# Blaok/soda

Hardware: AMD Instinct MI355X
Metric: stencil cells*iters/s, jacobi2d 8192x8192 iterate=100 (higher is better)
Workload: dtype f32; 1 GPU; jacobi2d float 8192x8192 iterate=100; kernel_family=march2d, decomposition=none, overlap=False, transport=none

## Files before the change

### soda_amd/codegen/hip/lower.py

```python
import dataclasses
import os
from typing import Dict, Optional, Sequence, Union

from soda_amd import core, util

from soda_amd.codegen.hip.module import (KernelDesc, Module, PassDesc,
                                         _check_native, runtime_text)
from soda_amd.codegen.hip.direct import DIRECT_BLOCK, add_direct_pass
from soda_amd.codegen.hip.ldswin import (add_ldswin_pass,
                                         ldswin_candidate, ldswin_pays,
                                         ldswin_supported)
from soda_amd.codegen.hip.march import (LANE_SHIFTS, MAX_FUSE_3D,
                                        MAX_FUSE_PRESERVE, MAX_SHIFT_TEMPS,
                                        MAX_UNROLL, REG_BUDGET, MarchConfig,
                                        add_march_pass, default_vec,
                                        march_supported)


MAX_TENSORS = 16
DEFAULT_FUSE = (13, 12, 8, 4)
SLIDING_SUMS = os.environ.get('SODA_HIP_SLIDE', '1') != '0'


STRATEGIES = ('auto', 'direct', 'march', 'ldswin')


@dataclasses.dataclass(kw_only=True, eq=False)
class LowerOptions:

  strategy: str = 'auto'
  fuse: Sequence[int] = (4,)
  vec: Optional[int] = None
  chunk_rows: Optional[int] = None
  prefetch: Optional[int] = None
  waves_x: int = 1
  waves_y: int = 1
  nt_store: Optional[bool] = None
  nt_load: Optional[bool] = None
  xcd_swizzle: bool = True
  edge_loads: bool = True
  tile_rows: Optional[int] = None
  lane_shift: Optional[str] = None
  min_waves: int = 0
  occupancy: int = 0
  pipe: Optional[int] = None
  pipe_rows: int = 2
  reg_budget: Optional[int] = None
  stamps: bool = False
  peel: Union[None, int, Dict[int, int]] = None
  align_lanes: Optional[int] = None
  xshare: Optional[bool] = None
  row_cells: Optional[int] = None
  windows: Optional[bool] = None
  inline: Optional[bool] = None

  def __post_init__(self):
    self.fuse = tuple(self.fuse)
    if self.inline is None:
      self.inline = os.environ.get('SODA_HIP_INLINE', '1') != '0'
    if self.windows is None:
      self.windows = os.environ.get('SODA_HIP_WINDOWS', '1') != '0'
    if self.xshare is None and os.environ.get('SODA_HIP_XSHARE'):
      self.xshare = os.environ['SODA_HIP_XSHARE'] == '1'
    if self.align_lanes is None and os.environ.get('SODA_HIP_ALIGN_LANES'):
      self.align_lanes = int(os.environ['SODA_HIP_ALIGN_LANES'])

  def resolved(self, dim: int, iterated: bool = True) -> 'LowerOptions':
    out = dataclasses.replace(self)
    if out.prefetch is None and dim == 3:
      out.prefetch = 1
    if out.nt_load is None:
      out.nt_load = dim != 3 and iterated
    if out.nt_store is None:
      out.nt_store = not iterated
    if out.tile_rows is None:
      out.tile_rows = 4
    return out


NARROW_STRIP_OPS = (48, 128)


def prefers_narrow_strips(stencil: core.Stencil) -> bool:
  if os.environ.get('SODA_HIP_NARROW', '1') == '0':
    return False
  if stencil.dim != 2 or stencil.iterate != 1:
    return False
  if any(str(t) != 'float' for t in stencil.symbol_table.values()):
    return False
  from soda_amd import ir as _ir
  work = sum(_ir.op_count(s.stmt.expr) +
             sum(_ir.op_count(l.expr) for l in s.stmt.let)
             for s in stencil.ordered_stages)
  return NARROW_STRIP_OPS[0] <= work < NARROW_STRIP_OPS[1]


# ... 66 lines not shown
    skip = ()
    if marching:
      skip = ((0, None),) + (((stencil.dim - 1, '+'),) if SLIDING_SUMS else ())
    derived = windows.decompose(stencil, skip=skip)
    if len(derived.symbol_table) + len(derived.param_stmts) <= MAX_TENSORS \
        and same_boxes(derived):
      stencil = derived
  from soda_amd.codegen.hip import exact
  stencil = exact.specialize(stencil)
  mod = Module(stencil)
  use_march = opts.strategy in ('auto', 'march') and \
      march_supported(stencil) is None
  if opts.strategy == 'march' and not use_march:
    raise util.SemanticError('march: %s' % march_supported(stencil))
  if use_march:
    vec0 = opts.vec or default_vec(stencil)
    iterable = (len(stencil.input_names) == len(stencil.output_names) and
                stencil.input_types == stencil.output_types)
    cap = stencil.iterate
    if stencil.dim == 3 and opts.strategy != 'march':
      cap = min(cap, MAX_FUSE_3D)
    if stencil.preserve_border and opts.strategy != 'march':
      cap = min(cap, MAX_FUSE_PRESERVE)
    depths = sorted({min(t, cap) for t in opts.fuse if iterable} - {0, 1},
                    reverse=True)

    def peel_for(t: int) -> int:
      if opts.peel is None:
        return -1
      if isinstance(opts.peel, dict):
        return int(opts.peel.get(t, -1))
      return int(opts.peel)

    def pipe_for(t: int) -> int:
      want = default_pipe(t) if opts.pipe is None else opts.pipe
      ok = (want > 1 and t > 1 and t % want == 0 and
            opts.waves_x * opts.waves_y == 1)
      return want if ok else 1

    out_bytes = min(t.size_in_bytes for t in stencil.output_types)

    def shift_for(t: int, xshare: int = 0) -> str:
      if opts.lane_shift is not None:
        return opts.lane_shift
      if xshare or pipe_for(t) > 1 or opts.waves_x * opts.waves_y != 1:
        return 'dpp'
      return default_lane_shift(t, stencil.dim)

    def config(t: int, vec: int, pf: Optional[int],
               rows: Optional[int] = None, xshare: int = 0) -> MarchConfig:
      shift = shift_for(t, xshare)
      if pf is None:
        pf = default_prefetch(t, shift)
      if opts.align_lanes is not None:
        align = opts.align_lanes
      else:
        align = max(1, 64 // (vec * out_bytes)) if opts.nt_store else 1
      cfg = MarchConfig(
          fused_iters=t, vec=vec, chunk_rows=opts.chunk_rows or 64,
          prefetch=pf, waves_x=opts.waves_x, waves_y=opts.waves_y,
          nt_store=opts.nt_store, nt_load=opts.nt_load,
          xcd_swizzle=opts.xcd_swizzle, edge_loads=opts.edge_loads,
          tile_rows=rows or opts.tile_rows, lane_shift=shift,
          min_waves=opts.min_waves, occupancy=opts.occupancy,
          pipe=pipe_for(t), pipe_rows=opts.pipe_rows, stamps=opts.stamps,
          peel=peel_for(t), align_lanes=align, xshare=xshare,
          xwindow=bool(opts.windows),
          slide=bool(opts.windows) and SLIDING_SUMS)
      cfg.chunk_fixed = opts.chunk_rows is not None
      return cfg

    budget = opts.reg_budget or REG_BUDGET
    first = default_prefetch(1) if stencil.dim == 2 and work < 128 else \
        (2 if stencil.dim == 2 else 1)
    pfs = [opts.prefetch] if opts.prefetch else [first, 2, 1]
    pfs = sorted(set(pfs), reverse=True)
    rows_list = [opts.tile_rows]
    vecs = []
    v = vec0
    while v >= 1:
      vecs.append(v)
      v //= 2
    chosen = None
    last_error = None
    for v in vecs:
      for rows in rows_list:
        for pf in pfs:
          trial = Module(stencil)
          try:
            est = add_march_pass(trial, config(1, v, pf, rows)).traffic_model[
                'est_window_regs']
          except util.SemanticError as e:
            last_error = e
            continue
          if chosen is None or est < chosen[0]:
            chosen = (est, v, pf, rows)
          if est <= budget:
            break
        if chosen and chosen[0] <= budget:
          break
      if chosen and chosen[0] <= budget:
# ... 38 lines not shown
```

### soda_amd/codegen/hip/march.py

```python
from typing import Dict, List, Optional, Tuple

from soda_amd import core, ir, util

from soda_amd.codegen.hip.module import KernelDesc, Module, PassDesc

MAX_UNROLL = 24
MAX_FUSE_PRESERVE = 8
MAX_FUSE_3D = 2
MAX_SHIFT_TEMPS = 64
REG_BUDGET = 160


class _Node:

  def __init__(self, key, ctype: str, stage: Optional[core.Stage], it: int):
    self.key = key
    self.ctype = ctype
    self.stage = stage
    self.it = it
    self.parents: Dict[str, '_Node'] = {}
    self.delay = 0
    self.first_use = None
    self.window = 1
    self.slots = 1
# ... 6 lines not shown
    self.keep: Optional[str] = None
    self.xs = False

  def tap_bounds(self, pname: str):
    dim = len(self.stage.st_idx)
    if pname in self.stage.taps:
      lo, hi = self.stage.tap_bounds(pname)
    else:
      lo, hi = (0,) * dim, (0,) * dim
    if pname == self.keep:
      lo = tuple(min(0, v) for v in lo)
      hi = tuple(max(0, v) for v in hi)
    return lo, hi

  @property
  def is_input(self) -> bool:
    return self.stage is None and self.mirror_of is None

  @property
  def fill_delay(self) -> int:
    if self.mirror_of is not None:
      return self.delay - MIRROR_PREFETCH
    return 0 if self.stage is None else self.delay

  @property
  def var(self) -> str:
    if self.mirror_of is not None:
      return 'm%d_%s' % (self.owner, self.mirror_of.var)
    if self.stage is None:
      return 'g_%s' % self.key[1]
    return 't%d_%s' % (self.it, self.stage.name)


LDS_PER_CU = 160 * 1024
MIRROR_PREFETCH = 1


LANE_SHIFTS = {'dpp': '', 'mixh': '_mixh'}


class MarchConfig:

  def __init__(self, *, fused_iters: int = 1, vec: int = 4, chunk_rows: int = 64,
               prefetch: int = 2, waves_x: int = 1, waves_y: int = 1,
               nt_store: bool = False, nt_load: bool = True,
               xcd_swizzle: bool = True, edge_loads: bool = True,
               tile_rows: int = 6, lane_shift: str = 'dpp',
               min_waves: int = 0, occupancy: int = 0,
               pipe: int = 1, pipe_rows: int = 4, stamps: bool = False,
               peel: int = -1, align_lanes: int = 1, xshare: int = 0,
               xwindow: bool = True, slide: bool = True):
    self.xwindow = xwindow
    self.slide = slide
    self.xshare = int(xshare)
    self.align_lanes = max(1, int(align_lanes))
    self.peel = int(peel)
    self.stamps = stamps
    self.pipe_rows = pipe_rows if pipe > 1 else 1
    self.pipe = pipe
    self.occupancy = occupancy
    self.min_waves = min_waves
    self.lane_shift = lane_shift
    self.fused_iters = fused_iters
    self.vec = vec
    self.chunk_rows = chunk_rows
    self.prefetch = prefetch
    self.waves_x = waves_x
    self.waves_y = waves_y
    self.nt_store = nt_store
    self.nt_load = nt_load
    self.xcd_swizzle = xcd_swizzle
    self.edge_loads = edge_loads
    self.tile_rows = tile_rows
    self.chunk_fixed = False

  def key(self) -> str:
    return ''.join((
        'T%d_V%d_P%d_W%dx%d_R%d' % (self.fused_iters, self.vec, self.prefetch,
                                    self.waves_x, self.waves_y, self.tile_rows),
        '_nts' if self.nt_store else '', '_ntl' if self.nt_load else '',
        '_xcd' if self.xcd_swizzle else '', '_edge' if self.edge_loads else '',
        LANE_SHIFTS[self.lane_shift],
        '_mw%d' % self.min_waves if self.min_waves else '',
        '_occ%d' % self.occupancy if self.occupancy else '',
        '_buf',
        '_pipe%dx%d' % (self.pipe, self.pipe_rows) if self.pipe > 1 else '',
        '_st' if self.stamps else '',
        '_k%d' % self.peel if self.peel >= 0 else '',
        '_al%d' % self.align_lanes if self.align_lanes > 1 else '',
        '_xs%d' % self.xshare if self.xshare else ''))


def default_vec(stencil: core.Stencil) -> int:
  widest = max(t.size_in_bytes for t in stencil.symbol_table.values())
  return max(1, 16 // widest)


def march_supported(stencil: core.Stencil) -> Optional[str]:
  if stencil.dim not in (2, 3):
    return 'the marching kernels need a 2- or 3-dimensional program'
  return None


def _build_chain(st: core.Stencil, T: int, pf: int, edge: Tuple[int, int],
                 pipe: int = 1, pipe_rows: int = 1, xshare: bool = False):
  dim = st.dim
  ax = dim - 1
  table = st.symbol_table
  per_wave = T // pipe
  nodes: List[_Node] = []
  inputs = {}
  for name in st.input_names:
    n = _Node(('in', name), table[name].c_type, None, -1)
    n.delay = pf
    n.margin = [-edge[0], -edge[1]]
# ... 436 lines not shown
      self.xs_stride = self.xs * 2 * self.xs_rows
      for n in self.xs_nodes:
        self.w('  __shared__ %s soda_xs_%s[%d];' %
               (n.ctype, n.var, 2 * self.xs_stride + 1))
      self.w('  if (threadIdx.x == 0) {')
      for n in self.xs_nodes:
        self.w('    soda_xs_%s[%d] = (%s)0;' % (n.var, 2 * self.xs_stride, n.ctype))
      self.w('  }')
      self.w('  soda_pipe_barrier();')
      self.w('  const int xs_wr = (wave * 2 + (lane == 0 ? 0 : 1)) * %d;' %
             self.xs_rows)
      self.w('  const int xs_nb = lane < 32 ? wave - 1 : wave + 1;')
      self.w('  const int xs_rd = (xs_nb >= 0 && xs_nb < %d && (lane & 31) < %d) ? '
             '(xs_nb * 2 + (lane < 32 ? 1 : 0)) * %d + (lane & 31) : %d;' %
             (self.xs, self.xs_rows, self.xs_rows, 2 * self.xs_stride))
    if self.n_edge:
      for i in range(self.n_edge):
        self.w('  const int ex%d = lane == 0 ? x0 - %d : x0 + %d;' %
          (i, 1 + i, self.V + i))
        self.w('  const bool edge_ok%d = edge_lane && ex%d >= 0 && ex%d < n0;' %
          (i, i, i))
        for es in sorted({self.esz[nme] for nme in self.inputs}):
          self.w('  const unsigned exb%d_%d = edge_ok%d ? (unsigned)ex%d * %du : '
            'SODA_OOB_X;' % (i, es, i, i, es))

    if self.st.preserve_border:
      for o in self.st.output_names:
        wlo, whi = self.st.interior_bounds(o)
        for e in range(self.V):
          self.w('  const bool keepx_%s_%d = !(a.origin[0] + x0 + %d >= %d && '
                 'a.origin[0] + x0 + %d < a.gextent[0] - %d);'
                 % (o, e, e, max(0, -wlo[0]), e, max(0, whi[0])))
    self.use_mix = self.cfg.lane_shift == 'mixh'
    self.slide: Dict[int, Tuple[str, Tuple[int, ...], int]] = {}
    if self.cfg.xwindow and self.cfg.slide and self.W == 1:
      from soda_amd.optimization import windows
      table = dict(self.st.symbol_table)
      for n in self.nodes:
        if n.stage is None or n.mirror_of is not None or n.keep is not None:
          continue
        m = windows._match(n.stage.stmt, table)
        if m is None or m[0] != '+' or m[2] != self.ax:
          continue
        off = tuple(a - b for a, b in zip(m[5], n.stage.st_idx))
        self.slide[id(n)] = (m[1], off, m[4])
    declared = set()
    for stage in self.st.ordered_stages:
      for line in self.mod.param_decls(stage):
        if line not in declared:
          declared.add(line)
          self.w(line)
    for n in self.nodes:
      if n.to_lds:
        self.w('  __shared__ %s soda_ring_%s[%d][%d][%d];' % (
            n.ctype, n.var, 2 * self.R, self.rows_in, 64 * self.V))
    self.nt_l = 'true' if self.cfg.nt_load else 'false'
    self.nt_s = 'true' if self.cfg.nt_store else 'false'

  def emit_decls(self, wv: int) -> None:
      for n in self.nodes:
        if n.owner != wv:
          continue
        if id(n) in self.slide:
          for j in self.rows_of(n):
            self.w('  int xa_%s_r%d[%d];' % (n.var, j, self.V))
            self.w('  soda_zero_frag<int, %d>(xa_%s_r%d);' % (self.V, n.var, j))
# ... 14 lines not shown
      if pin:
        for es in sorted({self.esz[nme] for nme in self.inputs}):
          self.w('      unsigned xb%dp = xb%d; asm volatile("" : "+v"(xb%dp));'
                 % (es, es, es))
      pinned = 'p' if pin else ''
      for es in sorted({self.esz[nme] for nme in self.inputs}):
        if self.dim == 2:
          self.w('      const unsigned ro%d = plane_ok ? (unsigned)(t - wlo) * '
            'pitch_b%d : SODA_OOB_ROW;' % (es, es))
        else:
          self.w('      const unsigned po%d = plane_ok ? (unsigned)(t - wlo) * '
            'pitch_b%d : SODA_OOB_X;' % (es, es))
          for j in sorted({j for n in self.inputs.values() for j in self.rows_of(n)}):
            self.w('      const unsigned ro%d_%d = po%d + yo%d_%d;' %
                   (es, j, es, es, j))
      for nme, n in self.inputs.items():
        s = self.slot_of(n, k, 0)
        for j in self.rows_of(n):
          es = self.esz[nme]
          ro = 'ro%d' % es if self.dim == 2 else 'ro%d_%d' % (es, j)
          reg = '%s_s%d_r%d' % (n.var, s, j)
          self.w('      soda_buf_load_frag<%s, %d, %s>(%s, r_%s, %s + xb%d%s);' %
            (n.ctype, self.V, self.nt_l, reg, nme, ro, es, pinned))
          for i in range(self.n_edge):
            self.w('      { %s e1[1]; soda_buf_load_frag<%s, 1, false>(e1, r_%s, %s + '
              'exb%d_%d); %s_e[%d] = e1[0]; }' %
              (n.ctype, n.ctype, nme, ro, i, es, reg, i))

  def _emit_wave(self, wv: int) -> None:
    if self.W > 1:
      self.w('  if (wave == %d) {  // iterations %d..%d of the chain' %
             (wv, wv * (self.T // self.W), (wv + 1) * (self.T // self.W) - 1))
    self.emit_decls(wv)
    self.w('  int tau = m_begin + (%d);' % (self.m_lo + self.lead))
    if wv == 0:
      for i in range(self.lead):
        self.w('    {  // prologue: loads of plane tau - %d' % (self.lead - i))
        self.emit_loads((i - self.lead) % self.U, 'tau - %d' % (self.lead - i))
        self.w('    }')
    self.w('  const int tau_end = m_end + %d;' % self.max_delay)
    if self.peeled:
      self.w('  {  // warm-up: %d row steps, stages enter as their rows start '
             'to matter' % self.peeled)
      for i in range(self.peeled):
        self._emit_tick(wv, i % self.U, step=i)
      self.w('  }')
      self.w('  tau += %d;' % self.peeled)
    for n in self.nodes:
      if id(n) in self.slide and n.owner == wv and not (
          self.peeled and self.stage_needed(n, self.peeled - 1)):
        self.w('  {  // sliding sum of %s: the rows its window holds now' % n.var)
        self.w('    const int t = tau;')
        self._shifted = {}
        self._wide = {}
        self._stage_mark = len(self.L)
        self._emit_stage(n, 0, slide_init='only')
        self.w('  }')
    self.w('  for (; tau < tau_end; tau += %d) {' % self.U)
    for k in range(self.U):
      self._emit_tick(wv, k)
    self.w('  }')
    if self.W > 1:
      self.w('  }')

  def _emit_tick(self, wv: int, k: int, step: Optional[int] = None) -> None:
    at = k if step is None else step
    self.w('    {  // tick %d of %d' % (k, self.U))

    if self.W > 1 and k % self.R == 0:
      self.w('      soda_pipe_barrier();')
    if wv == 0:
      self.emit_loads(k, 'tau + %d' % at, pin=step is not None)
    else:
      self.w('      const int t = tau + %d;' % at)
    for n in self.nodes:
      if n.mirror_of is not None and n.owner == wv:
        for j in self.rows_of(n):
          self.w('      soda_load_frag<%s, %d, false>(%s_s%d_r%d, &soda_ring_%s'
                 '[(t + %d) & %d][%d][lane * %d]);' %
                 (n.ctype, self.V, n.var, self.slot_of(n, k, 0), j,
                  n.mirror_of.var, self.R, 2 * self.R - 1, j, self.V))
    self._shifted: Dict[Tuple[str, int, int, int, int], str] = {}
    self._wide: Dict[str, str] = {}
    self._stage_mark = len(self.L)
    fresh_xs: List[Tuple[_Node, int]] = []
    if self.xs and wv == 0:
      for n in self.inputs.values():
        if n.xs:
          fresh_xs.append((n, self.slot_of(n, k, self.PF)))
      for n in self.nodes:
        if not n.xs:
          continue
        slot = self.slot_of(n, k - 1, self.PF if n.is_input else 0)
        self.w('      hv_%s_s%d = soda_xs_%s[xs_rd < %d ? xs_rd + ((t - 1) & 1) * %d '
               ': xs_rd];' % (n.var, slot, n.var, 2 * self.xs_stride,
                              self.xs_stride))
    for n in self.nodes:
      if n.stage is not None and n.owner == wv:
        if step is not None and not self.stage_needed(n, step):
          continue
        first = step is not None and (step == 0 or
                                      not self.stage_needed(n, step - 1))
        self._emit_stage(n, k, slide_init='first' if first else None)
        if n.xs:
          fresh_xs.append((n, self.slot_of(n, k, 0)))
    self.shift_temps = max(self.shift_temps, len(self._shifted))
    if fresh_xs:
      self.w('      if (edge_lane) {')
      for n, slot in fresh_xs:
        for jj, j in enumerate(self.rows_of(n)):
          reg = '%s_s%d_r%d' % (n.var, slot, j)
          self.w('        soda_xs_%s[xs_wr + (t & 1) * %d + %d] = lane == 0 ? %s[0] '
                 ': %s[%d];' % (n.var, self.xs_stride, jj, reg, reg, self.V - 1))
      self.w('      }')
      self.w('      soda_pipe_barrier();')
    self.w('    }')

  def _emit_stage(self, n: _Node, k: int,
                  slide_init: Optional[str] = None) -> None:
    stage = n.stage
    pre: List[str] = []
    early: List[str] = []

    def operand(pname: str, off: Tuple[int, ...], j: int, e: int, _n=n,
                _k=k, _pre=pre, _early=early) -> str:
      p = _n.parents[pname]
      age = _n.delay - off[self.ax] - p.fill_delay
      slot = self.slot_of(p, _k, age)
      row = j + (off[1] if self.dim == 3 else 0)
      if row < p.rmargin[0] or row >= self.rows_in - p.rmargin[1]:
        raise util.InternalError('march: row %d of %s is not held' %
                                 (row, p.var))
      reg = '%s_s%d_r%d' % (p.var, slot, row)
      c = e + off[0]
      lane_off, sub = c // self.V, c % self.V
      src = '%s[%d]' % (reg, sub)
      byte = p.ctype in ('uint8_t', 'int8_t')

      def wide(text: str, tag: str) -> str:
        if not byte:
          return text
        if tag not in self._wide:
          self._wide[tag] = 'w%d_%s' % (len(self._wide), tag)
          _pre.append('      const int %s = soda_wide(%s);' %
                      (self._wide[tag], text))
        return self._wide[tag]

      if lane_off == 0:
        return wide(src, '%s_e%d' % (reg, sub))
      key = (p.var, slot, row, sub, lane_off)
      if key not in self._shifted:
        tmp = 'sh_%s_e%d_%s%d' % (reg, sub, 'm' if lane_off < 0 else 'p',
                                  abs(lane_off))
        if (p.is_input and self.n_edge) or p.xs:
          if abs(lane_off) != 1:
            raise util.InternalError('march: edge loads reach one lane')
          ei = (-c - 1) if lane_off < 0 else (c - self.V)
          if p.xs:
            rr = row - p.rmargin[0] + (0 if lane_off < 0 else 32)
            old = ('soda_bcast(hv_%s_s%d, %d)' % (p.var, slot, rr)
                   if ei == 0 else '(%s)0' % p.ctype)
          else:
            old = '%s_e[%d]' % (reg, ei) if 0 <= ei < self.n_edge else \
                '(%s)0' % p.ctype
          expr = ('soda_lane_dn_or(%s, %s)' if lane_off < 0 else
                  'soda_lane_up_or(%s, %s)') % (src, old)
        elif self.use_mix and lane_off > 0:
          expr = src
          for _ in range(lane_off):
            expr = 'soda_lane_up32(%s)' % expr
        else:
          expr = src
          for _ in range(abs(lane_off)):
            expr = ('soda_lane_dn(%s)' if lane_off < 0 else
                    'soda_lane_up(%s)') % expr
        line = '      const %s %s = %s;' % (p.ctype, tmp, expr)
        early = self.use_mix and lane_off > 0 and (
            p.is_input or age > 0) and not (p.is_input and self.n_edge) \
            and not p.xs
        (_early if early else _pre).append(line)
        self._shifted[key] = tmp
      return wide(self._shifted[key], self._shifted[key])
# ... 152 lines not shown
                '%s(%s, (%s)%s)' % (fn, prev, pt, cells[i])
            body.append('        const %s %s = %s;' % (pt, name, expr))
            pre[i] = prev = name
          for e in range(e0, e0 + b):
            parts = ['xm_%s' % btag]
            if e < lo:
              parts.append(suf[e])
            if e + taps - 1 > hi:
              parts.append(pre[e + taps - 1])
            expr = parts[0]
            for q in parts[1:]:
              expr = '%s(%s, %s)' % (fn, expr, q)
            body.append('        %s = (%s)(%s);' % (dst[e], n.ctype, expr))
      body.append('      }')

  def _emit_store(self, n: _Node, oname: str, dst_slot: int) -> None:
    es = self.esz[oname]
    self.w('      {')
    self.w('        const int m = t - %d;' % n.delay)
    self.w('        const bool m_ok = m >= m_begin && m < m_end;')
    for j in self.store_rows(n):
      reg = '%s_s%d_r%d' % (n.var, dst_slot, j)
      if self.dim == 3:
        self.w('        soda_buf_store_frag<%s, %d, %s>(w_%s, (m_ok ? (unsigned)'
          '(m - m_begin) * pitch_b%d : SODA_OOB_X) + yo%d_%d + sxb%d, %s);' %
          (n.ctype, self.V, self.nt_s, oname, es, es, j, es, reg))
      else:
        self.w('        soda_buf_store_frag<%s, %d, %s>(w_%s, (m_ok ? '
          '(unsigned)(m - m_begin) * pitch_b%d : SODA_OOB_ROW) + sxb%d, '
          '%s);' % (n.ctype, self.V, self.nt_s, oname, es, es, reg))
    self.w('      }')

  def _finish(self) -> PassDesc:
    if self.shift_temps > MAX_SHIFT_TEMPS:
      raise util.SemanticError(
          'march: %d lane-shifted operands per row step (> %d); the taps reach '
          'too far along dim 0 for %d cells per lane' %
          (self.shift_temps, MAX_SHIFT_TEMPS, self.V))
    self.est_regs += self.shift_temps
    stages = [n for n in self.nodes if n.stage is not None]
    per_wave = []
    for wv in range(self.W):
      ops = 0.0
      for n in stages:
        if n.owner != wv:
          continue
        cost = sum(ir.op_count(l.expr) for l in n.stage.stmt.let) + \
            ir.op_count(n.stage.stmt.expr) + 0.5
        wide = 2.0 if n.ctype in ('double', 'int64_t', 'uint64_t') else 1.0
        ops += cost * wide * self.V * len(self.rows_of(n))
      per_wave.append(ops + 8.0)
    step_ops = max(per_wave)
    saved = sum(1 for i in range(self.peeled) for n in stages
                if not self.stage_needed(n, i)) / float(max(1, len(stages)))
    if self.dim == 2:
      tile = (self.strip_cells * (self.xs or self.wx),
              self.cfg.chunk_rows * self.cfg.waves_y)
    else:
      tile = (self.strip_cells * (self.xs or 1), self.tile_rows,
              self.cfg.chunk_rows)
    lds_pad = 0
    if self.cfg.occupancy:
      blocks_per_cu = max(1, 4 * self.cfg.occupancy // self.waves)
      lds_pad = min(65536, (LDS_PER_CU // (blocks_per_cu + 1)) // 1024 * 1024
                    + 1024)
    idx = self.mod.add_kernel(
        KernelDesc(self.name, (self.block, 1, 1), tile, lds_bytes=lds_pad,
                   note='%s %s' % (self.kind, self.cfg.key()),
                   tune=dict(axis=self.ax, waves_along=self.cfg.waves_y if self.dim == 2 else 1,
                             waves_per_block=self.waves, warm=self.warm,
                             fixed=self.cfg.chunk_fixed, occupancy=self.cfg.occupancy,
                             pipe=self.W, vec=self.V, step_ops=step_ops,
# ... 32 lines not shown
```

### soda_amd/csrc/soda_hip.cpp

```cpp
#include "soda_internal.h"

#include <hip/hiprtc.h>

#include <cmath>
#include <cstdlib>
#include <cstring>
#include <new>

namespace soda_detail {

thread_local std::string g_error;

int fail(int status, const std::string& what) {
  g_error = what;
  return status;
}

const std::string& last_error_text() { return g_error; }

int hip_fail(hipError_t e, const char* what) {
  char buf[512];
  snprintf(buf, sizeof buf, "%s: %s (%d)", what, hipGetErrorString(e), (int)e);
  g_error = buf;
  if (e == hipErrorOutOfMemory) return SODA_HIP_ERR_NOMEM;
// ... 266 lines not shown
      if (b.ptr) (void)hipFree(b.ptr);
  for (int i = 0; i < 2; ++i) {
    if (p->ev_pre[i]) (void)hipEventDestroy(p->ev_pre[i]);
    if (p->ev_bnd[i]) (void)hipEventDestroy(p->ev_bnd[i]);
  }
  if (p->side) (void)hipStreamDestroy(p->side);
  for (auto& st : p->hstream)
    if (st) (void)hipStreamDestroy(st);
  p->ring_in.release();
  p->ring_out.release();
  for (auto& b : p->band_out)
    if (b.ptr) (void)hipFree(b.ptr);
  for (auto& e : p->hevents) (void)hipEventDestroy(e);
  if (p->module) (void)hipModuleUnload(p->module);
  delete p;
  return SODA_HIP_OK;
}

namespace {

const int kSimds = 1024;
const double kHbmBytesPerNs = 6369.0;
const double kLaunchNs = 2547.0;
const double kWaveNs = 391.0;
const double kNormP = 2.708;
const int64_t kBufWindowMax = 1ll << 30;

int waves_per_simd(int vgprs) {
  int alloc = vgprs < 8 ? 8 : (vgprs + 7) / 8 * 8;
  int w = 512 / alloc;
  return w < 1 ? 1 : w > 8 ? 8 : w;
}

double issue_share(int64_t k) { return k == 1 ? 2.0 : k == 2 ? 1.2 : 1.0; }
double time_share(int64_t k) {
  return k == 1 ? 1.312 : k == 2 ? 1.475 : k == 3 ? 1.365 : 1.046;
}

int32_t tuned_chunk(const soda_hip_kernel_desc_t& d, const int32_t* tile,
                    const int32_t* extent, int dim, int64_t others) {
  const int axis = d.march_dim - 1;
  const int32_t n = extent[axis];
  const int wpb = (d.block[0] * d.block[1] * d.block[2] + 63) / 64;
  const int along = d.waves_along > 0 ? d.waves_along : 1;
  const bool load_only_warm = d.warm > 12 && d.warm_saved >= 0.75 * d.warm;
  const double warm = load_only_warm ? d.warm : d.warm - d.warm_saved;
  (void)tile; (void)dim;
  const int cap = waves_per_simd(d.vgprs);
  if (d.pipe > 1) {
    int32_t target = (int32_t)(3.5 * d.warm) > 64 ? (int32_t)(3.5 * d.warm) : 64;
    int64_t chunks = (n + target - 1) / target;
    if (chunks < 1) chunks = 1;
    const int64_t slots = (int64_t)kSimds * cap / d.pipe;
    int64_t blocks = others * chunks;
    if (blocks > slots * 0.975 && blocks < slots * 1.6) {
      chunks = (int64_t)(slots * 0.975) / others;
      if (chunks < 1) chunks = 1;
    }
    return (int32_t)((n + chunks - 1) / chunks);
  }
  const int k_min = d.warm <= 12 ? 4 : 2;
  double best_cost = 0;
  int32_t best = 0;
  for (int32_t chunk = n < 8 ? n : 8; chunk <= n;) {
    int64_t chunks = (n + chunk - 1) / chunk;
    int64_t blocks = others * ((chunks + along - 1) / along);
    int64_t waves = blocks * wpb;
    double cost;
    const int64_t slots = (int64_t)cap * kSimds;
    if (waves <= slots) {
      int64_t k = (waves + kSimds - 1) / kSimds;
      if (cap > 1) {
        if (k >= cap && waves > 0.975 * k * kSimds) ++k;
        if (k < k_min) k = k_min;
      }
      cost = k * issue_share(k) * (chunk + warm);
    } else {
      const int64_t full = waves / slots, rem = waves - full * slots;
      cost = full * cap * issue_share(cap) * (chunk + warm);
      if (rem > 0) {
        const int64_t rk = (rem + kSimds - 1) / kSimds;
// ... 50 lines not shown
    int32_t per_wave = g->tile[axis] / along;
    if (per_wave < 1) per_wave = 1;
    if (!d.chunk_fixed && d.vgprs > 0)
      per_wave = tuned_chunk(d, g->tile, extent, dim, others);
    if (d.window_extra >= 0) {
      int64_t plane = d.max_elem > 0 ? d.max_elem : 8;
      for (int i = 0; i < axis; ++i) plane *= extent[i];
      int64_t limit = kBufWindowMax / plane - d.window_extra;
      if (limit < 1) {
        snprintf(buf, sizeof buf,
                 "%s: one plane of this extent (%lld bytes) exceeds the 1 GiB "
                 "buffer window of the marching kernels; use the `direct` "
                 "strategy", d.name, (long long)plane);
        return fail(SODA_HIP_ERR_INVALID, buf);
      }
      if (per_wave > limit) {
        if (d.chunk_fixed) {
          snprintf(buf, sizeof buf,
                   "%s: chunks of %d planes exceed the 1 GiB buffer window on "
                   "this extent (at most %lld)", d.name, per_wave,
                   (long long)limit);
          return fail(SODA_HIP_ERR_INVALID, buf);
        }
        per_wave = (int32_t)limit;
      }
    }
    g->tile[axis] = per_wave * along;
    const int32_t n = extent[axis];
    const int64_t chunks = (n + per_wave - 1) / per_wave;
    const int64_t waves = others * ((chunks + along - 1) / along) * wpb;
    const int pipe = d.pipe > 0 ? d.pipe : 1;
    double steps = per_wave + d.warm - d.warm_saved;
    if (steps < 1) steps = 1;
    const int64_t slots = (int64_t)(d.vgprs > 0 ? waves_per_simd(d.vgprs) : 8) *
                          kSimds;
    const int64_t full = waves / slots, rem = waves - full * slots;
    double share = full * (double)(slots / kSimds) * time_share(slots / kSimds);
    if (rem > 0 || full == 0) {
      int64_t rk = (rem + kSimds - 1) / kSimds;
      if (rk < 1) rk = 1;
      share += rk * time_share(rk);
    }
    valu_ns = share * steps * d.step_ns / pipe;
    rows_factor = (per_wave + (double)d.warm) / per_wave;
    wave_ns = kWaveNs * (double)waves / kSimds;
  }
  if (d.step_ns > 0 || d.bytes_per_cell > 0) {
    const double lanes = d.lane_redundancy > 1 ? d.lane_redundancy : 1.0;
    const double bytes = cells * (double)d.bytes_per_cell *
                         (0.5 * lanes * rows_factor + 0.5);
    const double mem_ns = bytes / kHbmBytesPerNs;
    g->ns = pow(pow(valu_ns, kNormP) + pow(mem_ns, kNormP), 1.0 / kNormP) +
            kLaunchNs + wave_ns;
  }
  return SODA_HIP_OK;
}

int plan_geometry(const soda_hip_plan_t& plan, const int32_t* extent,
                  std::vector<Geometry>* geo, std::vector<double>* pass_ns) {
  geo->resize(plan.num_kernels);
  for (int k = 0; k < plan.num_kernels; ++k)
    if (int rc = kernel_geometry(plan.kernels[k], extent, plan.dim, &(*geo)[k]))
      return rc;
  pass_ns->assign(plan.num_passes, 0.0);
  for (int i = 0; i < plan.num_passes; ++i) {
    double t = 0;
    bool modelled = true;
// ... 1121 lines not shown
```

### soda_amd/csrc/soda_rt.h

```cpp

#ifdef __HIPCC_RTC__
typedef __INT8_TYPE__ int8_t;
typedef __UINT8_TYPE__ uint8_t;
typedef __INT16_TYPE__ int16_t;
typedef __UINT16_TYPE__ uint16_t;
typedef __INT32_TYPE__ int32_t;
typedef __UINT32_TYPE__ uint32_t;
typedef __INT64_TYPE__ int64_t;
typedef __UINT64_TYPE__ uint64_t;
#else
#include <hip/hip_runtime.h>
#include <stdint.h>
#endif

struct soda_hip_kargs_t {
  void* buf[16];
  int64_t stride[4];
  int32_t extent[4];
  int32_t ntile[4];
  int32_t tile[4];
  int32_t origin[4];
  int32_t gextent[4];
  int32_t skip_from;
  int32_t skip_count;
// ... 180 lines not shown
SODA_DEV int soda_swz_up32(int v) {
  return __builtin_amdgcn_ds_swizzle(v, SODA_SWZ_ROT_UP);
}

template <class T, int kSize = sizeof(T)>
struct soda_swz;
template <class T>
struct soda_swz<T, 4> {
  SODA_DEV T dn32(T v) { return __builtin_bit_cast(T, soda_swz_dn32(__builtin_bit_cast(int, v))); }
  SODA_DEV T up32(T v) { return __builtin_bit_cast(T, soda_swz_up32(__builtin_bit_cast(int, v))); }
};
template <class T>
struct soda_swz<T, 8> {
  struct pair { int lo, hi; };
#define SODA_SWZ_PAIR(fn)                          \
  SODA_DEV T fn(T v) {                             \
    pair p = __builtin_bit_cast(pair, v);          \
    p.lo = soda_swz_##fn(p.lo);                    \
    p.hi = soda_swz_##fn(p.hi);                    \
    return __builtin_bit_cast(T, p);               \
  }
  SODA_SWZ_PAIR(dn32) SODA_SWZ_PAIR(up32)
#undef SODA_SWZ_PAIR
};
template <class T>
struct soda_swz<T, 2> {
  SODA_DEV T dn32(T v) { return (T)soda_swz_dn32((int)v); }
  SODA_DEV T up32(T v) { return (T)soda_swz_up32((int)v); }
};
template <class T>
struct soda_swz<T, 1> : soda_swz<T, 2> {};
template <class T> SODA_DEV T soda_lane_dn32(T v) { return soda_swz<T>::dn32(v); }
template <class T> SODA_DEV T soda_lane_up32(T v) { return soda_swz<T>::up32(v); }

template <class T, int V>
struct soda_vec {
  typedef T type __attribute__((ext_vector_type(V)));
};

template <class T, int V, bool kNonTemporal = false>
SODA_DEV void soda_load_frag(T (&dst)[V], const T* __restrict__ p) {
  if constexpr (V == 1) {
    dst[0] = kNonTemporal ? __builtin_nontemporal_load(p) : *p;
  } else {
    typedef typename soda_vec<T, V>::type vec_t;
    const vec_t* vp = reinterpret_cast<const vec_t*>(p);
    const vec_t t = kNonTemporal ? __builtin_nontemporal_load(vp) : *vp;
#pragma unroll
    for (int e = 0; e < V; ++e) dst[e] = t[e];
  }
}

template <class T, int V>
SODA_DEV void soda_zero_frag(T (&dst)[V]) {
#pragma unroll
  for (int e = 0; e < V; ++e) dst[e] = (T)0;
}

template <class T, int V, bool kNonTemporal = false>
SODA_DEV void soda_store_frag(T* __restrict__ p, const T (&src)[V]) {
  if constexpr (V == 1) {
    if constexpr (kNonTemporal) __builtin_nontemporal_store(src[0], p);
    else *p = src[0];
  } else {
    typedef typename soda_vec<T, V>::type vec_t;
    vec_t t;
// ... 100 lines not shown
```

### soda_amd/isa.py

```python
import hashlib
import os
import re
import struct
import subprocess
from typing import Dict, List, Optional, Sequence, Tuple

OBJDUMP_CANDIDATES = ('/opt/rocm/lib/llvm/bin/llvm-objdump',
                      '/opt/rocm/llvm/bin/llvm-objdump')

SIMDS = 1024
PEAK_CLOCK_HZ = 2.4e9
CYCLES_PER_VALU = 2.0
VALU_PEAK_PER_S = SIMDS * PEAK_CLOCK_HZ / CYCLES_PER_VALU


def _sections(code: bytes):
  shoff, = struct.unpack_from('<Q', code, 0x28)
  shentsize, shnum = struct.unpack_from('<HH', code, 0x3A)
  return [struct.unpack_from('<IIQQQQIIQQ', code, shoff + i * shentsize)
          for i in range(shnum)]


def _symbols(code: bytes) -> Dict[str, Tuple[int, int, int, int]]:
  out = {}
# ... 104 lines not shown
  elif mnem.startswith(('buffer_', 'global_', 'flat_', 'scratch_')):
    kinds.append('vmem')
    kinds.append('vmem_store' if '_store' in mnem else 'vmem_load')
  elif mnem.startswith('s_waitcnt'):
    kinds.append('waitcnt')
  elif mnem.startswith('s_'):
    kinds.append('salu')
  return kinds


def _count(instrs) -> Dict[str, int]:
  out: Dict[str, int] = {'total': 0}
  for _, mnem, ops, _ in instrs:
    out['total'] += 1
    for k in _classify(mnem, ops):
      out[k] = out.get(k, 0) + 1
  return out


def static_profile(instrs) -> Dict[str, Dict[str, int]]:
  loops = [(t, a) for a, m, _, t in instrs if t is not None and t <= a]
  if not loops:
    return {'pre': _count(instrs), 'loop': {'total': 0}, 'post': {'total': 0},
            'loops': 0}
  head = min(t for t, _ in loops)
  tail = max(a for _, a in loops)
  pre = [i for i in instrs if i[0] < head]
  body = [i for i in instrs if head <= i[0] <= tail]
  post = [i for i in instrs if i[0] > tail]
  return {'pre': _count(pre), 'loop': _count(body), 'post': _count(post),
          'loops': len(loops)}


def march_waves(extent: Sequence[int], tile: Sequence[int], dim: int,
                tile_rows: int = 1) -> List[Tuple[int, int]]:
  ax = dim - 1
  others = -(-extent[0] // tile[0])
  if dim == 3:
    others *= -(-extent[1] // max(1, tile[1]))
  n, c = extent[ax], tile[ax]
  full, rest = divmod(n, c)
  out = [(others * full, c)] if full else []
  if rest:
    out.append((others, rest))
  return out


def march_valu_per_launch(profile: Dict[str, Dict[str, int]],
                          extent: Sequence[int], tile: Sequence[int], dim: int,
                          warm: int, peeled_steps: int, unroll: int,
                          kind: str = 'valu') -> float:
  pre = profile['pre'].get(kind, 0) + profile['post'].get(kind, 0)
  loop = profile['loop'].get(kind, 0)
  total = 0.0
  for waves, rows in march_waves(extent, tile, dim):
    trips = max(0, -(-(rows + warm - peeled_steps) // unroll))
    total += waves * (pre + trips * loop)
  return total


def module_static(module, code: bytes, tiles: Dict[str, Sequence[int]],
                  extent: Sequence[int]) -> Dict[str, dict]:
  dis = disassemble(code)
  dim = module.stencil.dim
  out = {}
  for k in module.kernels:
# ... 20 lines not shown
```

### soda_amd/runtime.py

```python
import ctypes
import hashlib
import os
from typing import Dict, Optional, Sequence

from soda_amd import core, util
from soda_amd.codegen.hip import lower

_HERE = os.path.dirname(os.path.abspath(__file__))
LIB_PATH = os.environ.get('SODA_HIP_LIBRARY') or \
    os.path.join(_HERE, 'libsoda_hip.so')
CACHE_DIR = os.environ.get('SODA_HIP_CACHE',
                           os.path.join(_HERE, '_jit_cache'))
ARCH = 'gfx950'
COMPILE_OPTIONS = ('--offload-arch=%s' % ARCH, '-O3', '-ffp-contract=off',
                   '-fno-slp-vectorize', '-fwrapv', '-std=c++17') + tuple(
                       os.environ.get('SODA_HIP_EXTRA_FLAGS', '').split())

MAX_DIM = 4
MAX_TENSORS = 16
MAX_KERNELS = 32
MAX_PASSES = 8
MAX_PASS_KERNELS = 16
MAX_PARAMS = 8
MAX_SLABS = 64
# ... 586 lines not shown
                                            '%s.hip' % stencil.app_name))
    for k in mod.kernels:
      if k.tune and k.tune.get('fused') == depth:
        r = res.get(k.name)
        return None if not r else (waves_per_simd(r['vgpr']), r['scratch'],
                                   r.get('code', 0))
    return None

  chosen = {}
  for depth, most in todo.items():
    base = probe(depth, 0)
    chosen[depth] = 0
    if base is None:
      continue
    for trips in range(most, 0, -1):
      got = probe(depth, trips)
      if got is None or got[0] < base[0] or got[1] > base[1]:
        continue
      if long_chunks.get(depth) and got[2] > ICACHE_BYTES >= base[2]:
        continue
      chosen[depth] = trips
      break
  try:
    os.makedirs(CACHE_DIR, exist_ok=True)
    tmp = '%s.%d.tmp' % (memo, os.getpid())
    with open(tmp, 'w') as f:
      json.dump(chosen, f)
    os.replace(tmp, memo)
  except OSError:
    pass
  return chosen


def select_shape(stencil: core.Stencil, opts: 'lower.LowerOptions',
                 extent: Optional[Sequence[int]] = None):
  import copy
  import json
  if opts.strategy not in ('auto', 'march') or stencil.iterate > 1:
    return None
  if min(t.size_in_bytes for t in stencil.symbol_table.values()) >= 4:
    return None
  base = copy.copy(opts)
  base.peel = 0
  mod0 = lower.lower(stencil, base)
  one = [k for k in mod0.kernels if k.tune and k.tune.get('fused') == 1 and
         'axis' in k.tune]
  if not one:
    return None
  chosen = int(one[0].tune.get('vec') or 1)
  want = int(opts.vec or lower.default_vec(stencil))
  if chosen >= want:
    return None
  key = hashlib.sha256(('shape2\0' + compiler_version() + '\0' +
                        '\0'.join(COMPILE_OPTIONS) + '\0%d\0' % want +
                        mod0.source).encode()).hexdigest()[:24]
  memo = os.path.join(CACHE_DIR, 'shape_%s.json' % key)
  try:
    with open(memo) as f:
      got = json.load(f)
    return tuple(got) if got else None
  except (OSError, ValueError):
    pass
  found = None
  vec = want
  while vec > chosen and found is None:
    for pf in (2, 1):
# ... 27 lines not shown
def resolve_options(stencil: core.Stencil,
                    opts: Optional['lower.LowerOptions'],
                    extent: Optional[Sequence[int]],
                    probe: bool = True) -> 'lower.LowerOptions':
  import copy
  out = copy.copy(opts) if opts is not None else lower.LowerOptions()
  if out.vec is None:
    out.vec = pick_vec(stencil, extent)
    if out.prefetch is None and out.strategy in ('auto', 'march') and \
        lower.prefers_narrow_strips(stencil):
      out.vec, out.prefetch = min(out.vec, 2), 4
  if out.row_cells is None and extent is not None:
    out.row_cells = int(extent[0])
  probing = probe and not os.environ.get('SODA_HIP_NO_PROBE')
  if probing and out.prefetch is None and out.reg_budget is None and \
      out.strategy in ('auto', 'march') and \
      lower.march_supported(stencil) is None:
    try:
      shape = select_shape(stencil, out, extent)
    except (util.SodaError, OSError):
      shape = None
    if shape:
      out.vec, out.prefetch = shape
      out.reg_budget = 1 << 20
  if out.peel is None and out.strategy in ('auto', 'march') and \
      lower.march_supported(stencil) is None:
    if not probe or os.environ.get('SODA_HIP_NO_PROBE'):
      out.peel = 0
    else:
      try:
        out.peel = select_peel(stencil, out, extent)
      except (util.SodaError, OSError):
        out.peel = 0
  return out


class Program:

  def __init__(self, stencil: core.Stencil,
               opts: Optional[lower.LowerOptions] = None, device: int = 0,
               extent: Optional[Sequence[int]] = None,
               calibrate: Optional[bool] = None,
               source_prefix: str = ''):
    self.stencil = stencil
    self.opts = resolve_options(stencil, opts, extent)
    self.device = device
    self.module = lower.lower(stencil, self.opts)
    self.code = compile_source(source_prefix + self.module.source,
                               '%s.hip' % stencil.app_name)
    self.resources = kernel_resources(self.code)
    self.plan = make_plan(self.module, self.resources)
    if extent is not None:
      self.geometry(extent)
    self._lib = library()
    self._handle = ctypes.c_void_p()
    check(
        self._lib.soda_hip_program_create(self.code, len(self.code),
                                          ctypes.byref(self.plan), device,
                                          ctypes.byref(self._handle)),
        'loading `%s` on GPU %d' % (stencil.app_name, device))
    if calibrate is False:
      check(self._lib.soda_hip_program_set_auto_calibrate(self._handle, 0),
            'set_auto_calibrate')
    if calibrate and extent is not None:
      self.calibrate(extent)

# ... 485 lines not shown
```

Baseline: 6106 billion cells*iters/s.

## Add optional early-issued lane-swizzle carries and LDS-aware occupancy model

Adds a swz_ahead option that hoists cross-lane up-shift swizzles for the next row step into the current step. The shifted operands are carried in registers, so swizzle latency can overlap with VALU work. An optional sched_barrier fence variant, an occupancy hold selector, and an ISA swizzle-cover analysis are also added. The runtime's wave-residency model now accounts for LDS limits. The default swz_ahead is 0, so the new path is disabled unless an environment variable is set; the only default-path change is the LDS-aware residency estimate used in planning.

```diff
diff --git a/soda_amd/codegen/hip/lower.py b/soda_amd/codegen/hip/lower.py
--- a/soda_amd/codegen/hip/lower.py
+++ b/soda_amd/codegen/hip/lower.py
@@ -20,6 +20,7 @@
 MAX_TENSORS = 16
 DEFAULT_FUSE = (13, 12, 8, 4)
 SLIDING_SUMS = os.environ.get('SODA_HIP_SLIDE', '1') != '0'
+DEFAULT_SWZ_AHEAD = 0
 
 
 STRATEGIES = ('auto', 'direct', 'march', 'ldswin')
@@ -42,7 +43,7 @@
   tile_rows: Optional[int] = None
   lane_shift: Optional[str] = None
   min_waves: int = 0
-  occupancy: int = 0
+  occupancy: Union[int, Dict[int, int]] = 0
   pipe: Optional[int] = None
   pipe_rows: int = 2
   reg_budget: Optional[int] = None
@@ -53,6 +54,7 @@
   row_cells: Optional[int] = None
   windows: Optional[bool] = None
   inline: Optional[bool] = None
+  swz_ahead: Optional[int] = None
 
   def __post_init__(self):
     self.fuse = tuple(self.fuse)
@@ -62,6 +64,9 @@
       self.windows = os.environ.get('SODA_HIP_WINDOWS', '1') != '0'
     if self.xshare is None and os.environ.get('SODA_HIP_XSHARE'):
       self.xshare = os.environ['SODA_HIP_XSHARE'] == '1'
+    if self.swz_ahead is None:
+      self.swz_ahead = int(os.environ.get('SODA_HIP_SWZ_AHEAD') or
+                           DEFAULT_SWZ_AHEAD)
     if self.align_lanes is None and os.environ.get('SODA_HIP_ALIGN_LANES'):
       self.align_lanes = int(os.environ['SODA_HIP_ALIGN_LANES'])
 
@@ -194,6 +199,11 @@
         return int(opts.peel.get(t, -1))
       return int(opts.peel)
 
+    def occupancy_for(t: int) -> int:
+      if isinstance(opts.occupancy, dict):
+        return int(opts.occupancy.get(t, 0))
+      return int(opts.occupancy)
+
     def pipe_for(t: int) -> int:
       want = default_pipe(t) if opts.pipe is None else opts.pipe
       ok = (want > 1 and t > 1 and t % want == 0 and
@@ -224,11 +234,12 @@
           nt_store=opts.nt_store, nt_load=opts.nt_load,
           xcd_swizzle=opts.xcd_swizzle, edge_loads=opts.edge_loads,
           tile_rows=rows or opts.tile_rows, lane_shift=shift,
-          min_waves=opts.min_waves, occupancy=opts.occupancy,
+          min_waves=opts.min_waves, occupancy=occupancy_for(t),
           pipe=pipe_for(t), pipe_rows=opts.pipe_rows, stamps=opts.stamps,
           peel=peel_for(t), align_lanes=align, xshare=xshare,
           xwindow=bool(opts.windows),
-          slide=bool(opts.windows) and SLIDING_SUMS)
+          slide=bool(opts.windows) and SLIDING_SUMS,
+          swz_ahead=opts.swz_ahead)
       cfg.chunk_fixed = opts.chunk_rows is not None
       return cfg
 
diff --git a/soda_amd/codegen/hip/march.py b/soda_amd/codegen/hip/march.py
--- a/soda_amd/codegen/hip/march.py
+++ b/soda_amd/codegen/hip/march.py
@@ -62,6 +62,18 @@
     return 't%d_%s' % (self.it, self.stage.name)
 
 
+class _Carry:
+
+  def __init__(self, src: _Node, row: int, sub: int, lanes: int, age: int):
+    self.src, self.row, self.sub, self.lanes = src, row, sub, lanes
+    self.age = age
+    self.var = 'cy_%s_r%d_e%d_p%d_a%d' % (src.var, row, sub, lanes, age)
+    self.users: List[_Node] = []
+
+  def at(self, k: int, unroll: int) -> str:
+    return '%s_k%d' % (self.var, k % unroll)
+
+
 LDS_PER_CU = 160 * 1024
 MIRROR_PREFETCH = 1
 
@@ -79,7 +91,9 @@
                min_waves: int = 0, occupancy: int = 0,
                pipe: int = 1, pipe_rows: int = 4, stamps: bool = False,
                peel: int = -1, align_lanes: int = 1, xshare: int = 0,
-               xwindow: bool = True, slide: bool = True):
+               xwindow: bool = True, slide: bool = True,
+               swz_ahead: int = 0):
+    self.swz_ahead = int(swz_ahead)
     self.xwindow = xwindow
     self.slide = slide
     self.xshare = int(xshare)
@@ -104,6 +118,10 @@
     self.tile_rows = tile_rows
     self.chunk_fixed = False
 
+  def ahead(self) -> int:
+    ok = self.lane_shift == 'mixh' and self.pipe == 1 and not self.xshare
+    return self.swz_ahead if ok else 0
+
   def key(self) -> str:
     return ''.join((
         'T%d_V%d_P%d_W%dx%d_R%d' % (self.fused_iters, self.vec, self.prefetch,
@@ -111,6 +129,7 @@
         '_nts' if self.nt_store else '', '_ntl' if self.nt_load else '',
         '_xcd' if self.xcd_swizzle else '', '_edge' if self.edge_loads else '',
         LANE_SHIFTS[self.lane_shift],
+        '_sa%d' % self.swz_ahead if self.ahead() else '',
         '_mw%d' % self.min_waves if self.min_waves else '',
         '_occ%d' % self.occupancy if self.occupancy else '',
         '_buf',
@@ -613,6 +632,8 @@
                  'a.origin[0] + x0 + %d < a.gextent[0] - %d);'
                  % (o, e, e, max(0, -wlo[0]), e, max(0, whi[0])))
     self.use_mix = self.cfg.lane_shift == 'mixh'
+    self.ahead = self.cfg.ahead()
+    self.carries: Dict[Tuple[str, int, int, int, int], _Carry] = {}
     self.slide: Dict[int, Tuple[str, Tuple[int, ...], int]] = {}
     if self.cfg.xwindow and self.cfg.slide and self.W == 1:
       from soda_amd.optimization import windows
@@ -693,6 +714,12 @@
       self.w('  if (wave == %d) {  // iterations %d..%d of the chain' %
              (wv, wv * (self.T // self.W), (wv + 1) * (self.T // self.W) - 1))
     self.emit_decls(wv)
+    if self.ahead:
+      self._plan_carries(wv)
+      for c in self.carries.values():
+        for k in range(self.U):
+          self.w('  %s %s = (%s)0;' % (c.src.ctype, c.at(k, self.U),
+                                       c.src.ctype))
     self.w('  int tau = m_begin + (%d);' % (self.m_lo + self.lead))
     if wv == 0:
       for i in range(self.lead):
@@ -700,6 +727,11 @@
         self.emit_loads((i - self.lead) % self.U, 'tau - %d' % (self.lead - i))
         self.w('    }')
     self.w('  const int tau_end = m_end + %d;' % self.max_delay)
+    if self.carries:
+      self.w('  {  // up-shifts for the first row step')
+      for n in self.nodes:
+        self._emit_carries(n, 0, 0 if self.peeled else None)
+      self.w('  }')
     if self.peeled:
       self.w('  {  // warm-up: %d row steps, stages enter as their rows start '
              'to matter' % self.peeled)
@@ -756,15 +788,21 @@
         self.w('      hv_%s_s%d = soda_xs_%s[xs_rd < %d ? xs_rd + ((t - 1) & 1) * %d '
                ': xs_rd];' % (n.var, slot, n.var, 2 * self.xs_stride,
                               self.xs_stride))
+    issued = set()
     for n in self.nodes:
       if n.stage is not None and n.owner == wv:
-        if step is not None and not self.stage_needed(n, step):
-          continue
-        first = step is not None and (step == 0 or
-                                      not self.stage_needed(n, step - 1))
-        self._emit_stage(n, k, slide_init='first' if first else None)
-        if n.xs:
-          fresh_xs.append((n, self.slot_of(n, k, 0)))
+        if step is None or self.stage_needed(n, step):
+          first = step is not None and (step == 0 or
+                                        not self.stage_needed(n, step - 1))
+          self._emit_stage(n, k, slide_init='first' if first else None)
+          if n.xs:
+            fresh_xs.append((n, self.slot_of(n, k, 0)))
+        if self.carries:
+          nxt = None if step is None or step + 1 >= self.peeled else step + 1
+          for p in [n] + [q for q in n.parents.values() if q.is_input]:
+            if id(p) not in issued:
+              issued.add(id(p))
+              self._emit_carries(p, k + 1, nxt)
     self.shift_temps = max(self.shift_temps, len(self._shifted))
     if fresh_xs:
       self.w('      if (edge_lane) {')
@@ -776,6 +814,29 @@
       self.w('      }')
       self.w('      soda_pipe_barrier();')
     self.w('    }')
+
+  def _plan_carries(self, wv: int) -> None:
+    text, self.L = self.L, []
+    self.w = self.L.append
+    self._shifted, self._wide, self._stage_mark = {}, {}, 0
+    for n in self.nodes:
+      if n.stage is not None and n.owner == wv:
+        self._emit_stage(n, 0)
+    self.L = text
+    self.w = self.L.append
+
+  def _emit_carries(self, p: _Node, k: int, step: Optional[int]) -> None:
+    for c in self.carries.values():
+      if c.src is not p:
+        continue
+      if step is not None and not any(self.stage_needed(u, step)
+                                      for u in c.users):
+        continue
+      expr = '%s_s%d_r%d[%d]' % (p.var, self.slot_of(p, k, c.age), c.row, c.sub)
+      for _ in range(c.lanes):
+        expr = 'soda_lane_up32_ahead(%s)' % expr
+      self.w('      %s = %s;%s' % (c.at(k, self.U), expr, ' soda_sched_fence();'
+                                   if self.ahead == 2 else ''))
 
   def _emit_stage(self, n: _Node, k: int,
                   slide_init: Optional[str] = None) -> None:
@@ -809,6 +870,15 @@
 
       if lane_off == 0:
         return wide(src, '%s_e%d' % (reg, sub))
+      if self.ahead and lane_off > 0 and id(_n) not in self.slide and \
+          not p.xs and not (p.is_input and self.n_edge) and (
+              age > (p.first_use or 0) if p.is_input else
+              p.stage is not None and age >= 1):
+        c = self.carries.setdefault((p.var, row, sub, lane_off, age),
+                                    _Carry(p, row, sub, lane_off, age))
+        if _n not in c.users:
+          c.users.append(_n)
+        return wide(c.at(_k, self.U), c.at(_k, self.U))
       key = (p.var, slot, row, sub, lane_off)
       if key not in self._shifted:
         tmp = 'sh_%s_e%d_%s%d' % (reg, sub, 'm' if lane_off < 0 else 'p',
@@ -1027,12 +1097,12 @@
     self.w('      }')
 
   def _finish(self) -> PassDesc:
-    if self.shift_temps > MAX_SHIFT_TEMPS:
+    if self.shift_temps + len(self.carries) > MAX_SHIFT_TEMPS:
       raise util.SemanticError(
           'march: %d lane-shifted operands per row step (> %d); the taps reach '
           'too far along dim 0 for %d cells per lane' %
-          (self.shift_temps, MAX_SHIFT_TEMPS, self.V))
-    self.est_regs += self.shift_temps
+          (self.shift_temps + len(self.carries), MAX_SHIFT_TEMPS, self.V))
+    self.est_regs += self.shift_temps + len(self.carries)
     stages = [n for n in self.nodes if n.stage is not None]
     per_wave = []
     for wv in range(self.W):
diff --git a/soda_amd/csrc/soda_hip.cpp b/soda_amd/csrc/soda_hip.cpp
--- a/soda_amd/csrc/soda_hip.cpp
+++ b/soda_amd/csrc/soda_hip.cpp
@@ -322,6 +322,16 @@
   return w < 1 ? 1 : w > 8 ? 8 : w;
 }
 
+int resident_waves(const soda_hip_kernel_desc_t& d) {
+  int cap = waves_per_simd(d.vgprs);
+  if (d.lds_bytes > 0) {
+    const int wpb = (d.block[0] * d.block[1] * d.block[2] + 63) / 64;
+    const int64_t by_lds = (160 * 1024 / d.lds_bytes) * (int64_t)wpb / 4;
+    if (by_lds < cap) cap = by_lds < 1 ? 1 : (int)by_lds;
+  }
+  return cap;
+}
+
 double issue_share(int64_t k) { return k == 1 ? 2.0 : k == 2 ? 1.2 : 1.0; }
 double time_share(int64_t k) {
   return k == 1 ? 1.312 : k == 2 ? 1.475 : k == 3 ? 1.365 : 1.046;
@@ -336,7 +346,7 @@
   const bool load_only_warm = d.warm > 12 && d.warm_saved >= 0.75 * d.warm;
   const double warm = load_only_warm ? d.warm : d.warm - d.warm_saved;
   (void)tile; (void)dim;
-  const int cap = waves_per_simd(d.vgprs);
+  const int cap = resident_waves(d);
   if (d.pipe > 1) {
     int32_t target = (int32_t)(3.5 * d.warm) > 64 ? (int32_t)(3.5 * d.warm) : 64;
     int64_t chunks = (n + target - 1) / target;
@@ -453,7 +463,7 @@
     const int pipe = d.pipe > 0 ? d.pipe : 1;
     double steps = per_wave + d.warm - d.warm_saved;
     if (steps < 1) steps = 1;
-    const int64_t slots = (int64_t)(d.vgprs > 0 ? waves_per_simd(d.vgprs) : 8) *
+    const int64_t slots = (int64_t)(d.vgprs > 0 ? resident_waves(d) : 8) *
                           kSimds;
     const int64_t full = waves / slots, rem = waves - full * slots;
     double share = full * (double)(slots / kSimds) * time_share(slots / kSimds);
diff --git a/soda_amd/csrc/soda_rt.h b/soda_amd/csrc/soda_rt.h
--- a/soda_amd/csrc/soda_rt.h
+++ b/soda_amd/csrc/soda_rt.h
@@ -236,6 +236,9 @@
 struct soda_swz<T, 1> : soda_swz<T, 2> {};
 template <class T> SODA_DEV T soda_lane_dn32(T v) { return soda_swz<T>::dn32(v); }
 template <class T> SODA_DEV T soda_lane_up32(T v) { return soda_swz<T>::up32(v); }
+
+template <class T> SODA_DEV T soda_lane_up32_ahead(T v) { return soda_swz<T>::up32(v); }
+SODA_DEV void soda_sched_fence() { __builtin_amdgcn_sched_barrier(0); }
 
 template <class T, int V>
 struct soda_vec {
diff --git a/soda_amd/isa.py b/soda_amd/isa.py
--- a/soda_amd/isa.py
+++ b/soda_amd/isa.py
@@ -160,6 +160,60 @@
           'loops': len(loops)}
 
 
+_LGKM = re.compile(r'lgkmcnt\((\d+)\)')
+
+
+def _lgkm_wait(ops: str) -> Optional[int]:
+  m = _LGKM.search(ops)
+  if m:
+    return int(m.group(1))
+  try:
+    return (int(ops.strip(), 0) >> 8) & 0xF
+  except ValueError:
+    return None
+
+
+def loop_body(instrs):
+  loops = [(t, a) for a, m, _, t in instrs if t is not None and t <= a]
+  if not loops:
+    return []
+  head = min(t for t, _ in loops)
+  tail = max(a for _, a in loops)
+  return [i for i in instrs if head <= i[0] <= tail]
+
+
+def swizzle_cover(instrs) -> List[int]:
+  body = loop_body(instrs)
+  flight: List[List[int]] = []
+  covers: Dict[int, int] = {}
+  valu = 0
+  for walk in range(2):
+    for idx, (_, mnem, ops, _) in enumerate(body):
+      if mnem.startswith('v_'):
+        valu += 1
+      elif mnem.startswith(('ds_', 's_load', 's_buffer_load')):
+        swz = mnem.startswith('ds_swizzle') and walk == 0
+        flight.append([valu, idx if swz else -1])
+      elif mnem.startswith('s_waitcnt'):
+        n = _lgkm_wait(ops)
+        if n is None:
+          continue
+        while len(flight) > n:
+          at, i = flight.pop(0)
+          if i >= 0:
+            covers[i] = valu - at
+  return [covers[i] for i in sorted(covers)]
+
+
+def cover_summary(covers: Sequence[int]) -> Dict[str, float]:
+  c = sorted(covers)
+  if not c:
+    return {'n': 0, 'min': 0, 'median': 0, 'max': 0}
+  mid = len(c) // 2
+  med = c[mid] if len(c) % 2 else 0.5 * (c[mid - 1] + c[mid])
+  return {'n': len(c), 'min': c[0], 'median': med, 'max': c[-1]}
+
+
 def march_waves(extent: Sequence[int], tile: Sequence[int], dim: int,
                 tile_rows: int = 1) -> List[Tuple[int, int]]:
   ax = dim - 1
diff --git a/soda_amd/runtime.py b/soda_amd/runtime.py
--- a/soda_amd/runtime.py
+++ b/soda_amd/runtime.py
@@ -642,6 +642,25 @@
   return chosen
 
 
+def select_hold(stencil: core.Stencil,
+                opts: 'lower.LowerOptions') -> Dict[int, int]:
+  import copy
+
+  def waves(o):
+    mod = lower.lower(stencil, o)
+    res = kernel_resources(compile_source(mod.source,
+                                          '%s.hip' % stencil.app_name))
+    return {k.tune['fused']: waves_per_simd(res[k.name]['vgpr'])
+            for k in mod.kernels
+            if k.tune and k.tune.get('lane_shift') == 'mixh' and
+            k.tune.get('waves_per_block') == 1 and k.name in res}
+
+  plain = copy.copy(opts)
+  plain.swz_ahead = 0
+  before, after = waves(plain), waves(opts)
+  return {t: before[t] for t in after if t in before and after[t] > before[t]}
+
+
 def select_shape(stencil: core.Stencil, opts: 'lower.LowerOptions',
                  extent: Optional[Sequence[int]] = None):
   import copy
@@ -735,6 +754,13 @@
         out.peel = select_peel(stencil, out, extent)
       except (util.SodaError, OSError):
         out.peel = 0
+  if out.swz_ahead and not out.occupancy and probing and \
+      out.strategy in ('auto', 'march') and \
+      lower.march_supported(stencil) is None:
+    try:
+      out.occupancy = select_hold(stencil, out)
+    except (util.SodaError, OSError):
+      pass
   return out
 
 
```

Result: slower. 6037 billion cells*iters/s (-1.1%).
